# NathanBWaters/playaid_core

Measured on AMD Instinct MI355X. Metric: 1080p frames/sec end-to-end, higher is better.
Workload: dtype f32; 1 GPU; configs[1]: 64 x 1080x1920 BGR frames per GPU per clip; parallelism=single GPU, lanes=2, ingest=raw BGR frames resident in HBM

## Files before the change

playaid_core_amd/csrc/stem_pool.hip:

```cpp
#include "tile_common.h"
#include "conv_rows.h"
#include "../../include/playaid_hip.h"
#include <cstring>

namespace pa {

namespace {

constexpr int IN_W = 134;
constexpr int POOL_W = 34;
constexpr int COUT = 64;
constexpr int KTOT = 224;

template <int FORM> struct StemGeom {
    static constexpr bool BF16 = FORM != 0;
    static constexpr int ROW_CH = BF16 ? IN_W / 2 : IN_W;
    static constexpr int PATCH_CH = 9 * ROW_CH;
    static constexpr int PASSES = (PATCH_CH + 255) / 256;
    static constexpr int STAGE_CH = PASSES * 256;
};

__device__ __forceinline__ f32x4 max4(f32x4 a, f32x4 b) {
    return f32x4{fmaxf(a.x, b.x), fmaxf(a.y, b.y), fmaxf(a.z, b.z), fmaxf(a.w, b.w)};
}

}

template <int FORM>
__global__ __launch_bounds__(256, 2) void stem_pool_kernel(const StemPoolParams p) {
    using G = StemGeom<FORM>;
    constexpr bool BF16 = FORM != 0;
    constexpr int NSL = FORM == 2 ? 3 : 1;
    constexpr int TS = 64;
    __shared__ __attribute__((aligned(16))) float lds[2 * G::STAGE_CH * 4 + 128 * TS];
    float* const tbuf = lds + 2 * G::STAGE_CH * 4;

    const int tid = threadIdx.x;
    const int lane = tid & 63;
    const int wave_id = __builtin_amdgcn_readfirstlane(tid >> 6);
    const int wm = wave_id >> 1;
    const int wn = wave_id & 1;
    const int lr = lane & 31;
    const int lh = lane >> 5;

    const int nwg = gridDim.x;
    const int wg = xcd_remap(blockIdx.x, nwg);
    const int runs_per_crop = 32 / p.run;
    const int runs_total = p.crops * runs_per_crop;

    const __amdgpu_buffer_rsrc_t x_rs = glds_rsrc(p.x);
#define SP_ISSUE(IMG, R, BUF)                                                                      \
    {                                                                                              \
        const int src_ = ((IMG) * IN_W + 4 * (R)) * G::ROW_CH;    \
        float* dst_ = lds + (BUF) * (G::STAGE_CH * 4) + wave_id * 256;                             \
        _Pragma("unroll") for (int i = 0; i < G::PASSES; ++i) {                                    \
            const int j = tid + 256 * i;                                                           \
            const int js = BF16 ? j : (j ^ ((j >> 4) & 1));                                        \
            if (j < G::PATCH_CH) glds16(x_rs, (src_ + js) * 16, 0, dst_ + i * 1024);               \
        }                                                                                          \
    }

    int run_id = wg;
    if (run_id >= runs_total) return;
    int crop = run_id / runs_per_crop;
    int r0 = (run_id - crop * runs_per_crop) * p.run;
    int rr = r0 > 0 ? r0 - 1 : 0;
    SP_ISSUE(crop, rr, 0);

    const int n = wn * 32 + lr;
    float bw[25][3];
    u32x4 bwh[NSL * 14];
    if constexpr (BF16) {
        const uint16_t* w = reinterpret_cast<const uint16_t*>(p.wgt) + (size_t)n * KTOT + 8 * lh;
#pragma unroll
        for (int g = 0; g < NSL * 14; ++g) bwh[g] = *reinterpret_cast<const u32x4*>(w + (size_t)(g / 14) * COUT * KTOT + (g % 14) * 16);
    } else {
        const float* w = reinterpret_cast<const float*>(p.wgt) + (size_t)n * KTOT;
#pragma unroll
        for (int st = 0; st < 25; ++st) {
            const int t0 = 2 * st, t1 = 2 * st + 1;
            const int o0 = (t0 / 7) * 32 + (t0 % 7) * 4, o1 = t1 < 49 ? (t1 / 7) * 32 + (t1 % 7) * 4 : -1;
            f32x4 v = *reinterpret_cast<const f32x4*>(w + (lh && o1 >= 0 ? o1 : o0));
            if (lh && o1 < 0) v = f32x4{0.f, 0.f, 0.f, 0.f};
            bw[st][0] = v.x;
            bw[st][1] = v.y;
            bw[st][2] = v.z;
        }
    }
    const float bias = p.bias[n];
    const int c_lane = BF16 ? (2 * wm) * G::ROW_CH + lr + lh : (2 * wm) * IN_W + 2 * lr;

    const int c4 = (tid & 15) * 4;
    f32x4 hprev[2] = {f32x4{0.f, 0.f, 0.f, 0.f}, f32x4{0.f, 0.f, 0.f, 0.f}};

    __syncthreads();
    int buf = 0;
    while (true) {
        int n_run = run_id, n_crop = crop, n_r0 = r0, n_rr = rr + 1;
        bool more = true;
        if (n_rr == r0 + p.run) {
            n_run = run_id + nwg;
            more = n_run < runs_total;
            if (more) {
                n_crop = n_run / runs_per_crop;
                n_r0 = (n_run - n_crop * runs_per_crop) * p.run;
                n_rr = n_r0 > 0 ? n_r0 - 1 : 0;
            }
        }
        if (more) SP_ISSUE(n_crop, n_rr, buf ^ 1);
        __builtin_amdgcn_sched_barrier(0);
        const float* patch = lds + buf * (G::STAGE_CH * 4);
        const bool warm = rr < r0;

        f32x16 acc[2];
#pragma unroll
        for (int mi = 0; mi < 2; ++mi)
#pragma unroll
            for (int e = 0; e < 16; ++e) acc[mi][e] = 0.f;

        if constexpr (BF16) {
            u32x4 af[2][2];
#define SP_FRAGS_H(SET, GG)                                                                        \
    {                                                                                              \
        _Pragma("unroll") for (int mi = 0; mi < 2; ++mi) {                                         \
            const int c = c_lane + ((GG) >> 1) * G::ROW_CH + 32 * mi + 2 * ((GG)&1);               \
            af[SET][mi] = *reinterpret_cast<const u32x4*>(patch + c * 4);                          \
        }                                                                                          \
    }
            if (FORM == 1 || !(warm && wm == 0)) {
            SP_FRAGS_H(0, 0);
#pragma unroll
            for (int t = 0; t < NSL * 14; ++t) {
                const int g = t % 14, sl = NSL - 1 - t / 14;
                if (t + 1 < NSL * 14) SP_FRAGS_H((t + 1) & 1, (t + 1) % 14);
                __builtin_amdgcn_sched_barrier(0);
#pragma unroll
                for (int mi = 0; mi < 2; ++mi)
                    acc[mi] = __builtin_amdgcn_mfma_f32_32x32x16_bf16(__builtin_bit_cast(bf16x8, af[t & 1][mi]),
                                                                      __builtin_bit_cast(bf16x8, bwh[sl * 14 + g]), acc[mi], 0, 0, 0);
                __builtin_amdgcn_sched_barrier(0);
            }
            }
#undef SP_FRAGS_H
        } else {
            f32x4 af[2][2];
#define SP_FRAGS(SET, ST)                                                                          \
    {                                                                                              \
        const int t0_ = 2 * (ST), t1_ = 2 * (ST) + 1 < 49 ? 2 * (ST) + 1 : 48;                      \
        const int off_ = lh ? (t1_ / 7) * IN_W + (t1_ % 7) : (t0_ / 7) * IN_W + (t0_ % 7);        \
        _Pragma("unroll") for (int mi = 0; mi < 2; ++mi) {                                         \
            const int c = c_lane + off_ + 64 * mi;                                                 \
            af[SET][mi] = *reinterpret_cast<const f32x4*>(patch + (c ^ ((c >> 4) & 1)) * 4);       \
        }                                                                                          \
    }
            if (!(warm && wm == 0)) {
            SP_FRAGS(0, 0);
#pragma unroll
            for (int g = 0; g < 25; ++g) {
#pragma unroll
                for (int mi = 0; mi < 2; ++mi) {
                    const f32x4 a4 = af[g & 1][mi];
                    acc[mi] = __builtin_amdgcn_mfma_f32_32x32x2f32(a4.x, bw[g][0], acc[mi], 0, 0, 0);
                    if (mi == 0) {
                        __builtin_amdgcn_sched_barrier(0);
                        if (g + 1 < 25) SP_FRAGS((g + 1) & 1, g + 1);
                        __builtin_amdgcn_sched_barrier(0);
                    }
                    acc[mi] = __builtin_amdgcn_mfma_f32_32x32x2f32(a4.y, bw[g][1], acc[mi], 0, 0, 0);
                    acc[mi] = __builtin_amdgcn_mfma_f32_32x32x2f32(a4.z, bw[g][2], acc[mi], 0, 0, 0);
                }
            }
            }
#undef SP_FRAGS
        }

#pragma unroll
        for (int mi = 0; mi < 2; ++mi)
#pragma unroll
            for (int e = 0; e < 16; ++e) {
                const int ox = mi * 32 + (e & 3) + 8 * (e >> 2) + 4 * lh;
                const float v = (FORM == 2 ? __fdiv_rn(acc[mi][e], 255.0f) : acc[mi][e]) + bias;
                tbuf[(wm * 64 + ox) * TS + n] = v > 0.f ? v : 0.f;
            }
        __syncthreads();
        {
            const bool store = rr >= r0;
#pragma unroll
            for (int i = 0; i < 2; ++i) {
                const int px = (tid >> 4) + 16 * i;
                f32x4 h[2];
#pragma unroll
                for (int row = 0; row < 2; ++row) {
                    const float* t = tbuf + (row * 64 + 2 * px) * TS + c4;
                    f32x4 m = max4(*reinterpret_cast<const f32x4*>(t), *reinterpret_cast<const f32x4*>(t + TS));
                    if (px > 0) m = max4(m, *reinterpret_cast<const f32x4*>(t - TS));
                    h[row] = m;
                }
                const f32x4 m = max4(max4(hprev[i], h[0]), h[1]);
                hprev[i] = h[1];
                if (store) {
                    const size_t o = (((size_t)crop * POOL_W + rr + 1) * POOL_W + px + 1) * COUT + c4;
                    if (p.out_bf16) {
                        *reinterpret_cast<uint2*>(reinterpret_cast<uint16_t*>(p.out) + o) = make_uint2(pack_bf16x2(m.x, m.y), pack_bf16x2(m.z, m.w));
                    } else {
                        *reinterpret_cast<f32x4*>(reinterpret_cast<float*>(p.out) + o) = m;
                    }
                }
            }
        }
        __syncthreads();
        if (!more) break;
        if (n_run != run_id) {
            hprev[0] = hprev[1] = f32x4{0.f, 0.f, 0.f, 0.f};
        }
        run_id = n_run; crop = n_crop; r0 = n_r0; rr = n_rr;
        buf ^= 1;
    }
#undef SP_ISSUE
}

hipError_t launch_stem_pool(const StemPoolParams& p_in, hipStream_t s) {
    StemPoolParams p = p_in;
    if (p.crops <= 0) return hipErrorInvalidValue;
    int per_crop = 1;
    while (per_crop < 8 && p.crops * per_crop < 512) per_crop *= 2;
    p.run = 32 / per_crop;
    const int runs = p.crops * per_crop;
    const int grid = runs < 512 ? runs : 512;
    if (p.in_bf16 == 2) {
        if (p.out_bf16) return hipErrorInvalidValue;
        hipLaunchKernelGGL(stem_pool_kernel<2>, dim3(grid), dim3(256), 0, s, p);
    } else if (p.in_bf16)
        hipLaunchKernelGGL(stem_pool_kernel<1>, dim3(grid), dim3(256), 0, s, p);
    else
        hipLaunchKernelGGL(stem_pool_kernel<0>, dim3(grid), dim3(256), 0, s, p);
    return hipGetLastError();
}

__global__ __launch_bounds__(256) void stem_int_pack_kernel(const uint8_t* __restrict__ crops, uint2* __restrict__ out, int n) {
    const size_t total = (size_t)n * 128 * 128;
    for (size_t i = (size_t)blockIdx.x * blockDim.x + threadIdx.x; i < total; i += (size_t)gridDim.x * blockDim.x) {
        const int img = (int)(i >> 14), pix = (int)(i & 16383);
        const int y = pix >> 7, x = pix & 127;
        const uint8_t* c = crops + i * 3;
        out[((size_t)img * IN_W + (y + 3)) * IN_W + (x + 3)] = make_uint2(u8_bf16x2(c[0], c[1]), u8_bf16x2(c[2], 0));
    }
}

}

extern "C" {

int pa_stem_int_pack_weights(const float* w_host, uint16_t* out_host) {
    if (!w_host || !out_host) return PA_ERR_INVALID_ARG;
    const size_t plane = (size_t)pa::COUT * pa::KTOT;
    memset(out_host, 0, 3 * plane * sizeof(uint16_t));
    for (int co = 0; co < pa::COUT; ++co)
        for (int t = 0; t < 49; ++t)
            for (int c = 0; c < 3; ++c) {
                float x = w_host[((size_t)co * 49 + t) * 3 + c];
                const size_t o = (size_t)co * pa::KTOT + (t / 7) * 32 + (t % 7) * 4 + c;
                for (int k = 0; k < 3; ++k) {
                    const uint16_t hq = pa::bf16_rne(x);
                    out_host[k * plane + o] = hq;
                    const uint32_t u = (uint32_t)hq << 16;
                    float f;
                    memcpy(&f, &u, 4);
                    x -= f;
                }
            }
    return PA_OK;
}

int pa_stem_int(const uint8_t* crops_u8, const void* w_slices, const float* bias, void* packed, float* out, int32_t n, void* stream) {
    if (!crops_u8 || !w_slices || !bias || !packed || !out || n < 1 || n > 8192) return PA_ERR_INVALID_ARG;
    auto misaligned = [](const void* q, unsigned long long m) { return (reinterpret_cast<unsigned long long>(q) & m) != 0; };
    if (misaligned(w_slices, 15) || misaligned(packed, 15) || misaligned(out, 15) || misaligned(bias, 3)) return PA_ERR_INVALID_ARG;
    hipStream_t s = static_cast<hipStream_t>(stream);
    int grid = (n * 16384 + 255) / 256;
    if (grid > 4096) grid = 4096;
    hipLaunchKernelGGL(pa::stem_int_pack_kernel, dim3(grid), dim3(256), 0, s, crops_u8, static_cast<uint2*>(packed), n);
    hipError_t e = hipGetLastError();
    if (e != hipSuccess) return PA_ERR_HIP;
    pa::StemPoolParams p;
    memset(&p, 0, sizeof(p));
    p.x = packed;
    p.wgt = w_slices;
    p.bias = bias;
    p.out = out;
    p.crops = n;
    p.in_bf16 = 2;
    e = pa::launch_stem_pool(p, s);
    return e == hipSuccess ? PA_OK : (e == hipErrorInvalidValue ? PA_ERR_INVALID_ARG : PA_ERR_HIP);
}

}
```

Measured before the change: 68760 frames/s.

## Defer stem pool epilogue after max-pool and interleave it with next tile's MFMAs

For the integer stem form, the divide-by-255, bias and ReLU move to after the 3x3 max-pool. Since these are monotonic, they now run once per pooled output instead of once per conv output. The pooling of each tile is split into small pieces that are interleaved between the next tile's MFMA instructions. The running row max is kept in LDS, and part of the weights move from registers to LDS to free VGPRs. This adds LDS traffic and scheduling complexity, and an env var selects the old paths.

Result: no change. 69200 frames/s (median of 6 runs) (+0.6%).

```diff
diff --git a/playaid_core_amd/csrc/stem_pool.hip b/playaid_core_amd/csrc/stem_pool.hip
--- a/playaid_core_amd/csrc/stem_pool.hip
+++ b/playaid_core_amd/csrc/stem_pool.hip
@@ -1,6 +1,7 @@
 #include "tile_common.h"
 #include "conv_rows.h"
 #include "../../include/playaid_hip.h"
+#include <cstdlib>
 #include <cstring>
 
 namespace pa {
@@ -26,14 +27,19 @@
 
 }
 
-template <int FORM>
+template <int FORM, int EPI>
 __global__ __launch_bounds__(256, 2) void stem_pool_kernel(const StemPoolParams p) {
+    static_assert(EPI == 0 || FORM == 2, "only the integer form has an epilogue worth moving");
     using G = StemGeom<FORM>;
     constexpr bool BF16 = FORM != 0;
     constexpr int NSL = FORM == 2 ? 3 : 1;
     constexpr int TS = 64;
-    __shared__ __attribute__((aligned(16))) float lds[2 * G::STAGE_CH * 4 + 128 * TS];
+    constexpr int NWL = EPI == 2 ? 6 : 0;
+    __shared__ __attribute__((aligned(16))) float lds[2 * G::STAGE_CH * 4 + 128 * TS + (EPI == 2 ? 2 * 256 * 4 + COUT + NWL * 2 * 64 * 4 : 0)];
     float* const tbuf = lds + 2 * G::STAGE_CH * 4;
+    float* const hp = tbuf + 128 * TS;
+    float* const lbias = hp + 2 * 256 * 4;
+    float* const wl = lbias + COUT;
 
     const int tid = threadIdx.x;
     const int lane = tid & 63;
@@ -73,7 +79,15 @@
     if constexpr (BF16) {
         const uint16_t* w = reinterpret_cast<const uint16_t*>(p.wgt) + (size_t)n * KTOT + 8 * lh;
 #pragma unroll
-        for (int g = 0; g < NSL * 14; ++g) bwh[g] = *reinterpret_cast<const u32x4*>(w + (size_t)(g / 14) * COUT * KTOT + (g % 14) * 16);
+        for (int g = 0; g < NSL * 14; ++g) {
+            const u32x4 v = *reinterpret_cast<const u32x4*>(w + (size_t)(g / 14) * COUT * KTOT + (g % 14) * 16);
+            const int t = g - (NSL - 1) * 14;
+            if (t >= 0 && t < NWL) {
+                if (wm == 0) *reinterpret_cast<u32x4*>(wl + ((t * 2 + wn) * 64 + lane) * 4) = v;
+            } else {
+                bwh[g] = v;
+            }
+        }
     } else {
         const float* w = reinterpret_cast<const float*>(p.wgt) + (size_t)n * KTOT;
 #pragma unroll
@@ -91,7 +105,49 @@
     const int c_lane = BF16 ? (2 * wm) * G::ROW_CH + lr + lh : (2 * wm) * IN_W + 2 * lr;
 
     const int c4 = (tid & 15) * 4;
-    f32x4 hprev[2] = {f32x4{0.f, 0.f, 0.f, 0.f}, f32x4{0.f, 0.f, 0.f, 0.f}};
+    constexpr float PAD = EPI ? -__builtin_inff() : 0.f;
+    f32x4 hprev[2] = {f32x4{PAD, PAD, PAD, PAD}, f32x4{PAD, PAD, PAD, PAD}};
+    const f32x4 bias4 = EPI == 1 ? f32x4{p.bias[c4], p.bias[c4 + 1], p.bias[c4 + 2], p.bias[c4 + 3]} : f32x4{0.f, 0.f, 0.f, 0.f};
+    if constexpr (EPI == 2) {
+        if (tid < COUT) lbias[tid] = p.bias[tid];
+        *reinterpret_cast<f32x4*>(hp + tid * 4) = *reinterpret_cast<f32x4*>(hp + (256 + tid) * 4) = f32x4{PAD, PAD, PAD, PAD};
+    }
+
+    int p_crop = 0, p_rr = 0;
+    bool p_store = false, p_reset = true;
+    f32x4 ra, rb, rm;
+    constexpr int NPIECE = 22;
+    auto piece = [&](const int K) __attribute__((always_inline)) {
+        const int i = K / 11, j = K % 11;
+        const int px = (tid >> 4) + 16 * i;
+        const float* t = tbuf + ((j >= 3 ? 64 : 0) + 2 * px) * TS + c4;
+        const int left = px > 0 ? -TS : 0;
+        float* const h = hp + (i * 256 + tid) * 4;
+        if (j == 0 || j == 3) {
+            ra = *reinterpret_cast<const f32x4*>(t);
+            rb = *reinterpret_cast<const f32x4*>(t + TS);
+        } else if (j == 1) {
+            rm = max4(ra, rb);
+            ra = *reinterpret_cast<const f32x4*>(t + left);
+            rb = *reinterpret_cast<const f32x4*>(h);
+        } else if (j == 2) {
+            rm = max4(rb, max4(rm, ra));
+        } else if (j == 4) {
+            ra = max4(ra, rb);
+            rb = *reinterpret_cast<const f32x4*>(t + left);
+        } else if (j == 5) {
+            ra = max4(ra, rb);
+            *reinterpret_cast<f32x4*>(h) = ra;
+            rm = max4(rm, ra);
+            rb = *reinterpret_cast<const f32x4*>(lbias + c4);
+        } else if (j < 10) {
+            const float v = __fdiv_rn(rm[j - 6], 255.0f) + rb[j - 6];
+            rm[j - 6] = v > 0.f ? v : 0.f;
+        } else if (p_store) {
+            const size_t o = (((size_t)p_crop * POOL_W + p_rr + 1) * POOL_W + px + 1) * COUT + c4;
+            *reinterpret_cast<f32x4*>(reinterpret_cast<float*>(p.out) + o) = rm;
+        }
+    };
 
     __syncthreads();
     int buf = 0;
@@ -129,17 +185,25 @@
     }
             if (FORM == 1 || !(warm && wm == 0)) {
             SP_FRAGS_H(0, 0);
+            u32x4 wt[2];
+            if (NWL) wt[0] = *reinterpret_cast<const u32x4*>(wl + (wn * 64 + lane) * 4);
 #pragma unroll
             for (int t = 0; t < NSL * 14; ++t) {
                 const int g = t % 14, sl = NSL - 1 - t / 14;
                 if (t + 1 < NSL * 14) SP_FRAGS_H((t + 1) & 1, (t + 1) % 14);
+                if (t + 1 < NWL) wt[(t + 1) & 1] = *reinterpret_cast<const u32x4*>(wl + (((t + 1) * 2 + wn) * 64 + lane) * 4);
                 __builtin_amdgcn_sched_barrier(0);
 #pragma unroll
-                for (int mi = 0; mi < 2; ++mi)
+                for (int mi = 0; mi < 2; ++mi) {
                     acc[mi] = __builtin_amdgcn_mfma_f32_32x32x16_bf16(__builtin_bit_cast(bf16x8, af[t & 1][mi]),
-                                                                      __builtin_bit_cast(bf16x8, bwh[sl * 14 + g]), acc[mi], 0, 0, 0);
+                                                                      __builtin_bit_cast(bf16x8, t < NWL ? wt[t & 1] : bwh[sl * 14 + g]), acc[mi], 0, 0, 0);
+                    if (EPI == 2 && 2 * t + mi >= 6 && (2 * t + mi - 6) % 3 == 0 && (2 * t + mi - 6) / 3 < NPIECE) piece((2 * t + mi - 6) / 3);
+                }
                 __builtin_amdgcn_sched_barrier(0);
             }
+            } else if (EPI == 2) {
+#pragma unroll
+                for (int k = 0; k < NPIECE; ++k) piece(k);
             }
 #undef SP_FRAGS_H
         } else {
@@ -174,15 +238,33 @@
 #undef SP_FRAGS
         }
 
+        if constexpr (EPI == 2) {
+            if (p_reset)
+                *reinterpret_cast<f32x4*>(hp + tid * 4) = *reinterpret_cast<f32x4*>(hp + (256 + tid) * 4) = f32x4{PAD, PAD, PAD, PAD};
+            __syncthreads();
+        }
 #pragma unroll
         for (int mi = 0; mi < 2; ++mi)
 #pragma unroll
             for (int e = 0; e < 16; ++e) {
                 const int ox = mi * 32 + (e & 3) + 8 * (e >> 2) + 4 * lh;
-                const float v = (FORM == 2 ? __fdiv_rn(acc[mi][e], 255.0f) : acc[mi][e]) + bias;
-                tbuf[(wm * 64 + ox) * TS + n] = v > 0.f ? v : 0.f;
+                if constexpr (EPI) {
+                    tbuf[(wm * 64 + ox) * TS + n] = acc[mi][e];
+                } else {
+                    const float v = (FORM == 2 ? __fdiv_rn(acc[mi][e], 255.0f) : acc[mi][e]) + bias;
+                    tbuf[(wm * 64 + ox) * TS + n] = v > 0.f ? v : 0.f;
+                }
             }
         __syncthreads();
+        if constexpr (EPI == 2) {
+            p_crop = crop; p_rr = rr;
+            p_store = rr >= r0;
+            p_reset = !more || n_run != run_id;
+            if (!more) break;
+            run_id = n_run; crop = n_crop; r0 = n_r0; rr = n_rr;
+            buf ^= 1;
+            continue;
+        }
         {
             const bool store = rr >= r0;
 #pragma unroll
@@ -196,9 +278,16 @@
                     if (px > 0) m = max4(m, *reinterpret_cast<const f32x4*>(t - TS));
                     h[row] = m;
                 }
-                const f32x4 m = max4(max4(hprev[i], h[0]), h[1]);
+                f32x4 m = max4(max4(hprev[i], h[0]), h[1]);
                 hprev[i] = h[1];
                 if (store) {
+                    if constexpr (EPI) {
+#pragma unroll
+                        for (int k = 0; k < 4; ++k) {
+                            const float v = __fdiv_rn(m[k], 255.0f) + bias4[k];
+                            m[k] = v > 0.f ? v : 0.f;
+                        }
+                    }
                     const size_t o = (((size_t)crop * POOL_W + rr + 1) * POOL_W + px + 1) * COUT + c4;
                     if (p.out_bf16) {
                         *reinterpret_cast<uint2*>(reinterpret_cast<uint16_t*>(p.out) + o) = make_uint2(pack_bf16x2(m.x, m.y), pack_bf16x2(m.z, m.w));
@@ -211,10 +300,14 @@
         __syncthreads();
         if (!more) break;
         if (n_run != run_id) {
-            hprev[0] = hprev[1] = f32x4{0.f, 0.f, 0.f, 0.f};
+            hprev[0] = hprev[1] = f32x4{PAD, PAD, PAD, PAD};
         }
         run_id = n_run; crop = n_crop; r0 = n_r0; rr = n_rr;
         buf ^= 1;
+    }
+    if constexpr (EPI == 2) {
+#pragma unroll
+        for (int k = 0; k < NPIECE; ++k) piece(k);
     }
 #undef SP_ISSUE
 }
@@ -229,11 +322,17 @@
     const int grid = runs < 512 ? runs : 512;
     if (p.in_bf16 == 2) {
         if (p.out_bf16) return hipErrorInvalidValue;
-        hipLaunchKernelGGL(stem_pool_kernel<2>, dim3(grid), dim3(256), 0, s, p);
+        static const int epi = getenv("PA_STEM_EPI") ? atoi(getenv("PA_STEM_EPI")) : 2;
+        if (epi == 2)
+            hipLaunchKernelGGL((stem_pool_kernel<2, 2>), dim3(grid), dim3(256), 0, s, p);
+        else if (epi)
+            hipLaunchKernelGGL((stem_pool_kernel<2, 1>), dim3(grid), dim3(256), 0, s, p);
+        else
+            hipLaunchKernelGGL((stem_pool_kernel<2, 0>), dim3(grid), dim3(256), 0, s, p);
     } else if (p.in_bf16)
-        hipLaunchKernelGGL(stem_pool_kernel<1>, dim3(grid), dim3(256), 0, s, p);
+        hipLaunchKernelGGL((stem_pool_kernel<1, 0>), dim3(grid), dim3(256), 0, s, p);
     else
-        hipLaunchKernelGGL(stem_pool_kernel<0>, dim3(grid), dim3(256), 0, s, p);
+        hipLaunchKernelGGL((stem_pool_kernel<0, 0>), dim3(grid), dim3(256), 0, s, p);
     return hipGetLastError();
 }
 
```
